# ctu-mrs/space_filling_forest_star

Measured on AMD Instinct MI355X. Metric: accepted node expansions/sec + collision checks/sec, dense_3D 6-DoF, higher is better.
Workload: dtype f64

## Files before the change

### space_filling_forest_star_amd/csrc/devforest.hip

```cpp
#include <hip/hip_runtime.h>
#include <stdint.h>
#include <stdlib.h>
#include "kernels.h"
#include "sff_geom.h"
#include "kernels_dev.h"

namespace sffk {

using namespace sffg;

__device__ __forceinline__ int record_words_dev(int nbcap) { return 6 + 4 * nbcap; }

__device__ __forceinline__ int lemire_pick(unsigned long long word, unsigned long long range) {
  const unsigned long long lo = word * range;
  const unsigned long long hi = __umul64hi(word, range);
  if (lo < range) {
    const unsigned long long thr = (0ULL - range) % range;
    if (lo < thr) return -1;
  }
  return (int)hi;
}

__device__ __forceinline__ int32_t* frontier_now(const DevForestView& f) { return f.ctrl->front_sel ? f.frontier2 : f.frontier; }
__device__ __forceinline__ int32_t* act_now(const DevForestView& f) { return f.ctrl->act_sel ? f.act_slot2 : f.act_slot; }

__device__ void round_begin_scalars(const DevForestView& f, DevCtrl* c) {
  const int cnt = c->act_cnt;
  int n = 0;
  if (c->round < f.threshold_misses && cnt > 0 && c->iter < f.max_iterations && !c->solved) {
    const int left = f.max_iterations - c->iter;
    n = cnt < left ? cnt : left;
  }
  c->n_act = n;
  if (n > 0) {
    if (c->n_nodes + n > f.node_cap - 8 || c->n_borders + n > f.border_cap) {
      c->fault = SFFK_FAULT_CAPACITY;
      c->halt = 1;
      c->n_act = 0;
    } else if ((unsigned long long)(c->n_borders + n) * 2ULL > f.bt_mask + 1ULL) {
      c->fault = SFFK_FAULT_BORDER_TABLE;
      c->halt = 1;
      c->n_act = 0;
    } else {
      c->round += 1;
      c->iter0 = c->iter;
      c->iter += n;
      c->N0 = c->n_nodes;
      c->words_base = c->cursor;
      c->cursor += (unsigned long long)f.words_per * (unsigned long long)n;
      c->rounds += 1;
      c->round_nodes += (unsigned long long)(c->n_nodes + n);
      c->round_queries += (unsigned long long)n;
    }
  }
}

#define WB_BLOCKS 64
__global__ __launch_bounds__(256) void k_wave_begin(DevForestView f) {
  __shared__ int s_last;
  __shared__ int s_scan[4];
  DevCtrl* c = f.ctrl;
  const unsigned long long tb0 = f.profile ? wall_clock64() : 0ULL;
  if (c->halt) {
    if (blockIdx.x == 0 && threadIdx.x == 0) { c->compact_from = 0; c->app_n = 0; }
    return;
  }
  if (c->in_wave) {
    if (blockIdx.x == 0 && threadIdx.x == 0) { c->compact_from = 0; c->app_n = 0; c->ord_valid = 0; round_begin_scalars(f, c); }
    return;
  }
  if (f.prio.n_heaps && !c->empty_frontier) return;
  const bool use_closed = c->closed_n > 0 && c->empty_frontier;
  const int pool = use_closed ? c->closed_n : c->frontier_n;
  int n_slots = f.wave < pool ? f.wave : pool;
  if (n_slots < 1) n_slots = 1;
  const int32_t* from = use_closed ? f.closed : frontier_now(f);
  int32_t* act = act_now(f);
  const unsigned long long cur = c->cursor;
  bool redraw = false;
  for (int sl = blockIdx.x * 256 + threadIdx.x; sl < n_slots; sl += gridDim.x * 256) {
    const unsigned long long wd = f.ring[(cur + (unsigned long long)sl) & f.ring_mask];
    const int pick = lemire_pick(wd, (unsigned long long)pool);
    if (pick < 0) redraw = true;
    else {
      const int node = from[pick];
      f.slot_node[sl] = node; f.slot_pos[sl] = pick;
      if (f.ord.hist) {
        const double* np = f.ord.pos + 6 * (size_t)node;
        const int cx = grid_coord((float)np[0], f.ord.ox, f.ord.inv_cell, f.ord.nx) >> f.ord.shift,
                  cy = grid_coord((float)np[1], f.ord.oy, f.ord.inv_cell, f.ord.ny) >> f.ord.shift,
                  cz = grid_coord((float)np[2], f.ord.oz, f.ord.inv_cell, f.ord.nz) >> f.ord.shift;
        const int key = (cz * f.ord.cny + cy) * f.ord.cnx + cx;
        f.ord.slot_key[sl] = key;
        f.ord.slot_rank[sl] = atomicAdd(&f.ord.hist[key], 1);
      }
    }
    act[sl] = sl;
  }
  if (redraw) atomicOr(&f.commit_seq[2], 1);
  __threadfence();
  __syncthreads();
  if (threadIdx.x == 0) s_last = atomicAdd(&f.commit_seq[1], 1) == (int)gridDim.x - 1;
  __syncthreads();
  if (!s_last) return;
  if (f.ord.hist) {
    constexpr int PERMAX = SFFK_ORD_BUCKETS / 256;
    const int nb = f.ord.n_buckets, per = (nb + 255) >> 8, lane = threadIdx.x & 63, wv = threadIdx.x >> 6;
    int v[PERMAX], sum = 0;
#pragma unroll
    for (int k = 0; k < PERMAX; ++k) {
      const int at = (int)threadIdx.x * per + k;
      v[k] = (k < per && at < nb) ? __hip_atomic_load(&f.ord.hist[at], __ATOMIC_RELAXED, __HIP_MEMORY_SCOPE_AGENT) : 0;
      sum += v[k];
    }
    int inc = sum;
    for (int off = 1; off < 64; off <<= 1) {
      const int o = __shfl_up(inc, off);
      if (lane >= off) inc += o;
    }
    if (lane == 63) s_scan[wv] = inc;
    __syncthreads();
    int run = inc - sum;
    for (int w = 0; w < wv; ++w) run += s_scan[w];
#pragma unroll
    for (int k = 0; k < PERMAX; ++k) {
      const int at = (int)threadIdx.x * per + k;
      if (k < per && at < nb) {
        f.ord.start[at] = run;
        run += v[k];
        f.ord.hist[at] = 0;
      }
    }
  }
  if (threadIdx.x != 0) return;
  c->ord_valid = (f.ord.hist && !__hip_atomic_load(&f.commit_seq[2], __ATOMIC_RELAXED, __HIP_MEMORY_SCOPE_AGENT)) ? 1 : 0;
  unsigned long long used = (unsigned long long)n_slots;
  if (__hip_atomic_load(&f.commit_seq[2], __ATOMIC_RELAXED, __HIP_MEMORY_SCOPE_AGENT)) {
    unsigned long long at = cur;
    for (int s = 0; s < n_slots; ++s) {
      int pick;
      do { pick = lemire_pick(f.ring[at & f.ring_mask], (unsigned long long)pool); ++at; } while (pick < 0);
      f.slot_node[s] = from[pick];
      f.slot_pos[s] = pick;
    }
    used = at - cur;
    c->redraws += 1;
  }
  f.commit_seq[1] = 0;
  f.commit_seq[2] = 0;
  c->compact_from = 0;
  c->app_n = 0;
  c->cursor = cur + used;
  c->n_slots = n_slots;
  c->act_cnt = n_slots;
  c->use_closed = use_closed ? 1 : 0;
  c->round = 0;
  c->in_wave = 1;
  c->waves += 1;
  c->prio_wave = 0;
  c->prio_n0 = c->n_nodes;
  round_begin_scalars(f, c);
  if (f.profile) c->wprof[6] += wall_clock64() - tb0;
}

__device__ __forceinline__ size_t border_slot(const DevForestView& f, unsigned long long key) {
  size_t h = (size_t)((key * 0x9E3779B97F4A7C15ULL) >> 17) & (size_t)f.bt_mask;
  while (true) {
    const unsigned long long cur = f.bt_key[h];
    if (cur == key) return h;
    if (cur == 0ULL) {
      const unsigned long long old = atomicCAS(&f.bt_key[h], 0ULL, key);
      if (old == 0ULL || old == key) return h;
    }
    h = (h + 1) & (size_t)f.bt_mask;
  }
}


#define KC_FAULT_SETTLE() asm volatile("s_waitcnt vmcnt(0)" ::: "memory")
#define KC_SPIN_LIMIT (1 << 20)
#define KC_ACC 0
#define KC_PREF 1
#define KC_WLO 2
#define KC_WHI 3
#define KC_POSTED 4
#define KC_OWN 5
#define KC_CNT 6
#define KC_DEP 12
#define KC_EVN 13

__device__ __forceinline__ unsigned long long kc_load(const unsigned long long* p) {
  return __hip_atomic_load(p, __ATOMIC_RELAXED, __HIP_MEMORY_SCOPE_AGENT);
}
__device__ __forceinline__ void kc_publish(unsigned long long* p, unsigned seq, unsigned v) {
  __hip_atomic_store(p, ((unsigned long long)seq << 32) | (unsigned long long)v, __ATOMIC_RELAXED, __HIP_MEMORY_SCOPE_AGENT);
}
__device__ __forceinline__ unsigned kc_wait(const unsigned long long* p, unsigned seq, int32_t* fault) {
  for (int spin = 0; spin < KC_SPIN_LIMIT; ++spin) {
    const unsigned long long v = kc_load(p);
    if ((unsigned)(v >> 32) == seq) return (unsigned)v;
    __builtin_amdgcn_s_sleep(1);
  }
  atomicOr(fault, 1);
  return 0u;
}
__device__ __forceinline__ unsigned long long kc_block_sum(unsigned long long v, unsigned long long* slot) {
  for (int off = 32; off > 0; off >>= 1) v += __shfl_xor(v, off);
  __syncthreads();
  if (threadIdx.x == 0) *slot = 0ULL;
  __syncthreads();
// ... 430 lines not shown
  }
  __syncthreads();
  for (int w = threadIdx.x; w < (int)(sizeof(DevCtrl) / 4); w += 1024)
    reinterpret_cast<int32_t*>(c)[w] = reinterpret_cast<const int32_t*>(&K)[w];
}

__device__ __forceinline__ void append_ord_store(const ResolveArgs& A, int ord_at, int next) {
  if (ord_at >= 0) (A.f.ctrl->app_act_sel ? A.f.ord.lst[0] : A.f.ord.lst[1])[ord_at] = next;
}
__device__ __forceinline__ int append_one(const ResolveArgs& A, int i, int& slot_out, int& ord_at, int part = 0) {
  ord_at = -1;
  const DevForestView& f = A.f;
  const DevCtrl* c = f.ctrl;
  const int n = c->app_n;
  slot_out = -1;
  if (n <= 0) return -1;
  const int act_cnt = c->app_act_cnt;
  const int32_t* act_old = c->app_act_sel ? f.act_slot2 : f.act_slot;
  int32_t* act_new = c->app_act_sel ? f.act_slot : f.act_slot2;
  const bool wave_over = c->n_act == 0 && !c->halt && c->in_wave && !c->use_closed;
  const bool ord_on = f.ord.hist && c->ord_valid;
  auto claim = [&](int e, int slot) {
    const int nd = f.slot_node[slot];
    atomicMin(&f.claim[nd], e);
    f.ulist[e] = nd;
  };
  if (wave_over && i == 0 && part != 1) f.ctrl->claims_done = 1;
  if (i >= n) {
    if (i < act_cnt && part != 1) {
      const int e = (c->act_cnt - (act_cnt - n)) + (i - n), slot = act_old[i];
      act_new[e] = slot;
      if (wave_over) claim(e, slot);
    }
    return -1;
  }
  const unsigned long long w = f.w_acc[i >> 6];
  const int rank = f.acc_pref[i >> 6] + __popcll(w & ((1ULL << (i & 63)) - 1ULL));
  if (!((w >> (i & 63)) & 1ULL)) {
    auto ord_append = [&](int slot) {
      const int sub = f.ord.slot_pos[slot] >> 6;
      const bool first = c->app_act_sel != 0;
      ord_at = sub * 64 + atomicAdd(&(first ? f.ord.cnt[0] : f.ord.cnt[1])[sub * SFFK_ORD_CNT_STRIDE], 1);
    };
    if (part == 1) {
      if (ord_on) { ord_append(act_old[i]); append_ord_store(A, ord_at, i - rank); }
      return -1;
    }
    slot_out = act_old[i];
    act_new[i - rank] = slot_out;
    if (ord_on && part == 0) ord_append(slot_out);
    if (wave_over) claim(i - rank, slot_out);
    return i - rank;
  }
  if (A.star || part == 2) return -1;
  const int N0 = c->app_N0, fn0 = c->app_fn0;
  int32_t* const frontier = frontier_now(f);
  const int id = N0 + rank;
  const int ex = A.parent[i];
  const double* p = A.newpos + 6 * (size_t)i;
  const size_t o = (size_t)id;
  GridItem it;
  for (int k = 0; k < 6; ++k) it.p[k] = p[k];
  it.id = id;
  it.tree = A.st.tree[ex];
  it.pad[0] = it.pad[1] = 0;
  A.st.x[o] = (float)p[0]; A.st.y[o] = (float)p[1]; A.st.z[o] = (float)p[2];
  A.st.yaw[o] = (float)p[3]; A.st.pitch[o] = (float)p[4]; A.st.roll[o] = (float)p[5];
  for (int k = 0; k < 6; ++k) A.st.pos[6 * o + k] = p[k];
  A.st.tree[o] = it.tree;
  const double pd = A.pdist[i];
  f.parent[o] = ex;
  f.d_closest[o] = pd;
  f.d_root[o] = pd + f.d_root[ex];
  f.iter[o] = (uint32_t)(c->iter0_app + i + 1);
  f.nflag[o] = f.prio.n_heaps ? 0 : 2;
  if (!f.prio.n_heaps) frontier[fn0 + rank] = id;
  grid_put(A.g, it);
  return -1;
}
__device__ void border_finalize(const ResolveArgs& A, int b) {
  __shared__ unsigned long long s_bsum;
  __shared__ int s_bown;
  const DevForestView& f = A.f;
  DevCtrl* c = f.ctrl;
  const int n = c->app_n;
  if (n <= 0 || A.star) return;
  const int nwg = (n + 63) >> 6;
  if (b >= nwg) return;
  const unsigned seq = (unsigned)f.commit_seq[0];
  const unsigned long long stamp_hi = c->epoch << 32;
  const int Tb = f.temp_base, nb0 = c->app_nb0;
  const unsigned long long we = f.w_ev[b];
  unsigned long long* pub = f.wg_pub + (size_t)b * SFFK_PUB_WORDS;
  const int tid = threadIdx.x;
  bool own = false;
  int e_i = 0;
  unsigned long long wo = 0ULL;
  if (tid < 64) {
    if ((we >> tid) & 1ULL) {
      e_i = b * 64 + tid;
      const unsigned long long owner = __hip_atomic_load(&f.bt_val[f.ev_h[e_i]], __ATOMIC_RELAXED, __HIP_MEMORY_SCOPE_AGENT);
      own = owner == (stamp_hi | (unsigned long long)(uint32_t)e_i);
    }
    wo = __ballot(own);
    if (tid == 0) { s_bown = __popcll(wo); kc_publish(pub + KC_OWN, seq, (unsigned)__popcll(wo)); }
  }
  __syncthreads();
  const int n_own = s_bown;
  const bool last = b == nwg - 1;
  if (n_own == 0 && !last) return;
  unsigned long long pe = 0;
  for (int t = tid; t < b; t += 256) pe += kc_wait(f.wg_pub + (size_t)t * SFFK_PUB_WORDS + KC_OWN, seq, f.commit_seq + 6);
  for (int off = 32; off > 0; off >>= 1) pe += __shfl_xor(pe, off);
  if (tid == 0) s_bsum = 0ULL;
  __syncthreads();
  if ((tid & 63) == 0 && pe) atomicAdd(&s_bsum, pe);
  __syncthreads();
  const int ev_pref = (int)s_bsum;
  if (own) {
    const int at = nb0 + ev_pref + __popcll(wo & ((1ULL << tid) - 1ULL));
    double pn[6], pe6[6], dn;
    int ta;
    const int raw = f.ev_raw[e_i], e_nb = f.ev_nb[e_i], e_ex = A.parent[e_i];
    if (raw >= Tb) {
      const int j = raw - Tb;
      for (int q = 0; q < 6; ++q) pn[q] = A.newpos[6 * (size_t)j + q];
      dn = A.pdist[j] + f.d_root[A.parent[j]];
      ta = A.st.tree[A.parent[j]];
    } else {
      for (int q = 0; q < 6; ++q) pn[q] = A.st.pos[6 * (size_t)e_nb + q];
      dn = f.d_root[e_nb];
      ta = A.st.tree[e_nb];
    }
    const int tb = A.st.tree[e_ex];
    f.b_n1[at] = e_nb < e_ex ? e_nb : e_ex; f.b_n2[at] = e_nb < e_ex ? e_ex : e_nb;
    f.b_ta[at] = ta < tb ? ta : tb; f.b_tb[at] = ta < tb ? tb : ta;
    for (int q = 0; q < 6; ++q) pe6[q] = A.st.pos[6 * (size_t)e_ex + q];
    f.b_dist[at] = dn + f.d_root[e_ex] + dist6(pn, pe6);
    f.pair[(size_t)ta * f.n_trees + tb] = 1;
    f.pair[(size_t)tb * f.n_trees + ta] = 1;
  }
  if (last && tid == 0) c->n_borders = nb0 + ev_pref + n_own;
}
__global__ __launch_bounds__(256) void k_append(ResolveArgs A, int append_blocks) {
  if ((int)blockIdx.x >= append_blocks) { border_finalize(A, (int)blockIdx.x - append_blocks); return; }
  int slot, ord_at;
  const int next = append_one(A, blockIdx.x * 256 + threadIdx.x, slot, ord_at);
  append_ord_store(A, ord_at, next);
}
__global__ __launch_bounds__(256) void k_append_sample(ResolveArgs A, SampleLaunch P, int append_blocks) {
  if ((int)blockIdx.x >= 2 * append_blocks) { border_finalize(A, (int)blockIdx.x - 2 * append_blocks); return; }
  const int nb = append_blocks;
  const bool sampler = (int)blockIdx.x >= nb;
  const int tid = ((int)blockIdx.x - (sampler ? nb : 0)) * 256 + threadIdx.x;
  int slot, ord_at;
  if (!sampler) { (void)append_one(A, tid, slot, ord_at, 1); return; }
  const int next = append_one(A, tid, slot, ord_at, 2);
  sample_steer_one(tid, next, slot < 0 ? -2 : slot, P);
  append_ord_store(A, ord_at, next);
}

__device__ void wave_end_control(const DevForestView& f, DevCtrl* c, int removed, int fn, bool from_closed, int n_fail,
                                 const int32_t* grid_ovf, const int32_t* tgrid_ovf, const unsigned long long* star_s) {
  c->closed_n += removed;
  if (f.prio.n_heaps) {
    c->compact_from = 0;
    c->empty_frontier = c->prio_all_empty;
  } else {
    c->compact_from = removed > 0 ? fn : 0;
    c->frontier_n = fn - removed;
    if (removed > 0) c->front_sel ^= 1;
    c->empty_frontier = c->frontier_n == 0 ? 1 : 0;
  }
  if (!c->solved && c->empty_frontier && f.goal_id < 0) {
    const int R = f.n_trees;
    int reached = 1;
    for (int t = 0; t < R; ++t) f.claim[t] = t == 0 ? 1 : 0;
    bool grew = true;
    while (grew) {
      grew = false;
      for (int a = 0; a < R; ++a) {
        if (f.claim[a] != 1) continue;
        f.claim[a] = 2;
        for (int b = 0; b < R; ++b)
          if (f.claim[b] == 0 && f.pair[(size_t)a * R + b]) { f.claim[b] = 1; ++reached; grew = true; }
      }
    }
    for (int t = 0; t < R; ++t) f.claim[t] = 0x7fffffff;
    c->solved = reached == R ? 1 : 0;
  }
  c->claims_done = 0;
  c->clear_n = from_closed ? 0 : n_fail;
  const bool budget = f.node_budget > 0 && c->n_nodes >= f.node_budget;
  c->terminated = (c->solved || c->iter >= f.max_iterations || budget) ? 1 : 0;
  c->halt = c->terminated;
  if (f.commit_seq[6]) { c->fault = SFFK_FAULT_INTERNAL; c->halt = 1; }
  c->in_wave = 0;
  c->n_act = 0;
  c->grid_ovf = grid_ovf[0];
  c->tgrid_ovf = tgrid_ovf[0];
  if (star_s) {
    c->collide_calls += star_s[0]; c->path_free_calls += star_s[1];
    c->star_rounds += star_s[2]; c->star_passes += star_s[3]; c->star_members += star_s[4]; c->star_rewires += star_s[5];
  }
}

#define KW_CNT 15
__device__ void status_publish(const DevForestView& f) {
  if (!f.host_status || threadIdx.x >= 64) return;
  DevCtrl* c = f.ctrl;
  const int sq = __hip_atomic_load(&c->status_seq, __ATOMIC_RELAXED, __HIP_MEMORY_SCOPE_AGENT);
  int32_t* dst = reinterpret_cast<int32_t*>(f.host_status + (sq & (SFFK_STATUS_RING - 1)));
// ... 235 lines not shown
```

### space_filling_forest_star_amd/csrc/devprio.hip

```cpp
#include <hip/hip_runtime.h>
#include <stdint.h>
#include "kernels.h"
#include "sff_geom.h"
#include "kernels_dev.h"
#include "prio_heap_dev.h"

namespace sffk {

using namespace sffg;

__device__ __forceinline__ int prio_lemire(unsigned long long word, unsigned long long range) {
  const unsigned long long lo = word * range;
  const unsigned long long hi = __umul64hi(word, range);
  if (lo < range) {
    const unsigned long long thr = (0ULL - range) % range;
    if (lo < thr) return -1;
  }
  return (int)hi;
}

#ifdef SFFK_PRIO_DEBUG
__device__ unsigned long long g_prio_dbg[16];
#endif
__device__ __forceinline__ int32_t* prio_act_now(const DevForestView& f) { return f.ctrl->act_sel ? f.act_slot2 : f.act_slot; }
// ... 68 lines not shown
  refill();
  auto next_word = [&]() -> unsigned long long {
    if (at - w_lo >= 128ULL) refill();
    const unsigned long long w = s_w[at - w_lo];
    ++at;
    return w;
  };
  auto draw_int = [&](int range) -> int {
    int v;
    do { v = prio_lemire(next_word(), (unsigned long long)range); } while (v < 0);
    return v;
  };
  int32_t* act = prio_act_now(f);
  int made = 0;
  int my_t = 0, my_h = 0, my_i = 0;
  for (int s = 0; s < n_slots; ++s) {
    if (total_ne == 0) break;
    if (at - w_lo >= 96ULL) refill();
    int t;
    do { t = draw_int(T); } while (s_tne[t] == 0);
    const int b0 = P.base[t], nh = P.base[t + 1] - b0;
    int hp;
    do { hp = draw_int(nh); } while (s_sz[b0 + hp] == 0);
    const int size = s_sz[b0 + hp];
    int idx = -1;
    if (!(uniform_real(next_word(), 0.0, 1.0) <= P.bias)) idx = draw_int(size);
    __builtin_amdgcn_wave_barrier();
    if (lane == 0) {
      s_sz[b0 + hp] = size - 1;
      if (size == 1) s_tne[t] -= 1;
    }
    __builtin_amdgcn_wave_barrier();
    if (size == 1) total_ne -= 1;
    if ((s & 63) == lane) { my_t = t; my_h = hp; my_i = idx; }
    if ((s & 63) == 63) {
      const int o = s - 63 + lane;
      P.slot_tree[o] = my_t; P.slot_heap[o] = my_h; P.slot_idx[o] = my_i; act[o] = o;
    }
    ++made;
  }
  if ((made & 63) != 0 && lane < (made & 63)) {
    const int o = (made & ~63) + lane;
    P.slot_tree[o] = my_t; P.slot_heap[o] = my_h; P.slot_idx[o] = my_i; act[o] = o;
  }
  if (lane == 0) {
    c->compact_from = 0;
    c->app_n = 0;
    c->cursor = at;
    c->n_slots = made;
    c->act_cnt = made;
    c->use_closed = 0;
    c->round = 0;
    c->in_wave = 1;
    c->waves += 1;
    c->prio_wave = 1;
    c->prio_gen = (int32_t)c->waves;
    c->prio_n0 = c->n_nodes;
    prio_round_begin(f, c);
  }
}


#define PP_COIN_WORDS ((4 * 64 * SFFK_DEV_MAX_GROUPS + 4096) / 32)
__global__ __launch_bounds__(1024) void k_prio_plan(DevForestView f) {
  __shared__ int s_sz[SFFK_PRIO_MAX_HEAPS];
  __shared__ int s_cnt[SFFK_PRIO_MAX_HEAPS];
  __shared__ unsigned int s_coin[PP_COIN_WORDS];
  __shared__ int s_fn[1024][4];
  __shared__ int s_bad, s_pool, s_used;
  DevCtrl* c = f.ctrl;
  const PrioView& P = f.prio;
  const int tid = threadIdx.x, lane = tid & 63;
  if (c->halt || c->in_wave || !P.plan) return;
  const int H = P.n_heaps, T = f.n_trees;
  for (int h = tid; h < H; h += 1024) { s_sz[h] = P.size[h]; s_cnt[h] = 0; }
  if (tid == 0) { s_bad = 0; s_pool = 0; s_used = -1; }
  __syncthreads();
  if (tid < T && P.base[tid + 1] > P.base[tid]) atomicAdd(&s_pool, s_sz[P.base[tid]]);
  __syncthreads();
  int n_slots = f.wave < s_pool ? f.wave : s_pool;
  if (n_slots < 1) n_slots = 1;
  const int M = 4 * n_slots + 8;
  int bk = (M + 1023) / 1024;
  if (bk < 4) bk = 4;
  const int span = 1024 * bk + 64;
  const unsigned long long cur = c->cursor;
  for (int p0 = 0; p0 < span; p0 += 8 * 1024) {
    unsigned long long w[8];
    for (int j = 0; j < 8; ++j) {
      const int p = p0 + j * 1024 + tid;
      w[j] = f.ring[(cur + (unsigned long long)(p < M ? p : M - 1)) & f.ring_mask];
    }
    for (int j = 0; j < 8; ++j) {
      const int p = p0 + j * 1024 + tid;
      const bool coin = p < M && !(uniform_real(w[j], 0.0, 1.0) <= P.bias);
      const unsigned long long m = __ballot(coin);
      if (lane == 0 && p < span && (p >> 5) + 1 < PP_COIN_WORDS) { s_coin[p >> 5] = (unsigned int)m; s_coin[(p >> 5) + 1] = (unsigned int)(m >> 32); }
    }
  }
  __syncthreads();
  auto hop = [&](int p) -> int { return p + 3 + (int)((s_coin[(p + 2) >> 5] >> ((p + 2) & 31)) & 1u); };
  const int lo = tid * bk, hi = lo + bk;
  for (int e = 0; e < 4; ++e) {
    int p = lo + e, n = 0;
    while (p < hi) { p = hop(p); ++n; }
    s_fn[tid][e] = (n << 2) | (p - hi);
// ... 2 lines not shown
  for (int d = 1; d < 1024; d <<= 1) {
    int g[4];
    for (int e = 0; e < 4; ++e) g[e] = s_fn[tid][e];
    if (tid >= d) {
      int r[4];
      for (int e = 0; e < 4; ++e) {
        const int first = s_fn[tid - d][e];
        const int then = g[first & 3];
        r[e] = (((first >> 2) + (then >> 2)) << 2) | (then & 3);
      }
      for (int e = 0; e < 4; ++e) g[e] = r[e];
    }
    __syncthreads();
    for (int e = 0; e < 4; ++e) s_fn[tid][e] = g[e];
    __syncthreads();
  }
  int p = lo, s = 0;
  if (tid > 0) { const int before = s_fn[tid - 1][0]; p = lo + (before & 3); s = before >> 2; }
  int32_t* act = prio_act_now(f);
  while (p < hi && s <= n_slots) {
    if (s == n_slots) { s_used = p; break; }
    const unsigned long long w0 = f.ring[(cur + (unsigned long long)p) & f.ring_mask];
    const unsigned long long w1 = f.ring[(cur + (unsigned long long)p + 1ULL) & f.ring_mask];
    const int nx = hop(p);
    bool bad = false;
    int t = prio_lemire(w0, (unsigned long long)T), hp = 0, idx = -1;
    unsigned long long w3 = 0ULL;
    if (t < 0) { bad = true; t = 0; }
    else {
      const int b0 = P.base[t], nh = P.base[t + 1] - b0;
      hp = nh > 0 ? prio_lemire(w1, (unsigned long long)nh) : -1;
      if (hp < 0) { bad = true; hp = 0; }
      else {
        atomicAdd(&s_cnt[b0 + hp], 1);
        if (nx - p == 4) { idx = -2; w3 = f.ring[(cur + (unsigned long long)p + 3ULL) & f.ring_mask]; }
      }
    }
    if (bad) s_bad = 1;
    P.slot_tree[s] = t; P.slot_heap[s] = hp; P.slot_idx[s] = idx; P.slot_word[s] = w3; act[s] = s;
    p = nx; ++s;
  }
  __syncthreads();
  for (int h = tid; h < H; h += 1024) if (s_cnt[h] > s_sz[h]) s_bad = 1;
  __syncthreads();
  if (s_bad || s_used < 0 || tid != 0) return;
  c->compact_from = 0;
  c->app_n = 0;
  c->cursor = cur + (unsigned long long)s_used;
  c->n_slots = n_slots;
  c->act_cnt = n_slots;
  c->use_closed = 0;
  c->round = 0;
  c->in_wave = 1;
  c->waves += 1;
  c->prio_wave = 1;
  c->prio_gen = (int32_t)c->waves;
  c->prio_n0 = c->n_nodes;
  prio_round_begin(f, c);
}

#define PG_CHUNK 2048
__device__ __forceinline__ int block_excl_scan_256(int v, int* s_w, int* total) {
  const int lane = threadIdx.x & 63, w = threadIdx.x >> 6;
  int x = v;
  for (int d = 1; d < 64; d <<= 1) { const int y = __shfl_up(x, d); if (lane >= d) x += y; }
  __syncthreads();
  if (lane == 63) s_w[w] = x;
  __syncthreads();
  int before = 0, sum = 0;
  for (int i = 0; i < 4; ++i) { if (i < w) before += s_w[i]; sum += s_w[i]; }
  *total = sum;
  return before + x - v;
}

__global__ __launch_bounds__(256) void k_prio_pops(DevForestView f) {
  __shared__ int s_slot[PG_CHUNK];
  __shared__ int s_idx[PG_CHUNK];
  __shared__ unsigned long long s_word[PG_CHUNK];
  __shared__ int s_w[4];
  const DevCtrl* c = f.ctrl;
  const PrioView& P = f.prio;
  const int h = blockIdx.x, tid = threadIdx.x, lane = tid & 63;
  if (!c->prio_wave || !c->in_wave || P.gen[h] == c->prio_gen) return;
  int t = 0;
  while (P.base[t + 1] <= h) ++t;
  const int hp = h - P.base[t];
  const int n_slots = c->n_slots;
  HeapRef hr = heap_of(P, h);
  for (int c0 = 0; c0 < n_slots; c0 += PG_CHUNK) {
    int st_[8], sh_[8];
    for (int j = 0; j < 8; ++j) {
      const int s = c0 + tid * 8 + j;
      const int sc = s < n_slots ? s : n_slots - 1;
      const int a_ = P.slot_tree[sc], b_ = P.slot_heap[sc];
      st_[j] = s < n_slots ? a_ : -1;
      sh_[j] = s < n_slots ? b_ : -1;
    }
    int cnt = 0;
    for (int j = 0; j < 8; ++j) cnt += (st_[j] == t && sh_[j] == hp) ? 1 : 0;
    int total;
    int at = block_excl_scan_256(cnt, s_w, &total);
    for (int j = 0; j < 8; ++j)
      if (st_[j] == t && sh_[j] == hp) {
        const int s = c0 + tid * 8 + j;
        const int idx = P.slot_idx[s];
        s_slot[at] = s; s_idx[at] = idx; s_word[at] = idx == -2 ? P.slot_word[s] : 0ULL;
// ... 160 lines not shown
```

### space_filling_forest_star_amd/csrc/kernels.h

```cpp
#pragma once
#include <hip/hip_runtime.h>
#include <stdint.h>

#include "knobs.h"

namespace sffk {

struct NodeStoreView {
  const float* x;
  const float* y;
  const float* z;
  const float* yaw;
  const float* pitch;
  const float* roll;
  const int32_t* tree;
  const double* pos;
};

struct NodeStoreMut {
  float *x, *y, *z, *yaw, *pitch, *roll;
  int32_t* tree;
  double* pos;
};

// ... 73 lines not shown
  int clear_n[3];
  const int32_t* tg_start;
  const int32_t* tg_list;
  double tg_org[3];
  double tg_inv;
  int tg_n[3];
};
void launch_tgrid_build(hipStream_t s, const EnvView& env, int32_t* cnt_or_start, int32_t* list, bool fill);
struct ClearBuildArgs {
  double thr_pose, thr_edge;
  double pose_lo[3], pose_hi[3];
  double edge_lo[3], edge_hi[3];
};
void launch_clear_build(hipStream_t s, const EnvView& env, const ClearBuildArgs& P, uint32_t* bits_pose, uint32_t* bits_edge,
                        long long n_cells);

struct RobotView {
  const double* tri;
  int n_tri;
  double center[3];
  double radius;
  double lo[3], hi[3];
};

struct DevCtrl {
  int32_t n_act;
  int32_t halt;
  int32_t n_nodes, iter, round, in_wave;
  int32_t n_slots, frontier_n, closed_n, use_closed;
  int32_t terminated, solved, empty_frontier, fault;
  int32_t N0, iter0, n_borders, n_unsettled;
  int32_t fault_pending, redraws, grid_ovf, tgrid_ovf;
  int32_t front_sel;
  int32_t compact_from;
  int32_t act_sel, act_cnt;
  int32_t app_n, app_N0, app_fn0, app_act_sel;
  int32_t iter0_app, app_act_cnt;
  int32_t claims_done;
  int32_t clear_n;
  unsigned long long cursor;
  unsigned long long words_base;
  unsigned long long collide_calls, path_free_calls, nn_queries;
  unsigned long long poses_executed, segments_executed, samples_executed;
  unsigned long long waves, rounds, round_nodes, round_queries;
  unsigned long long epoch;
  unsigned long long work_items;
  unsigned long long prof[8];
  unsigned long long q_t0, q_t1, q_ticks, q_launches;
  unsigned long long wprof[8];
  int32_t prio_n0, prio_wave, prio_all_empty, prio_gen;
  unsigned long long star_rounds, star_passes, star_members, star_rewires;
  int32_t ord_valid;
  int32_t app_nb0;
  int32_t status_seq, status_pad;
  unsigned long long spec_steps, spec_evaluated, spec_committed;
  int32_t spec_stalled, spec_pad;
};
#define SFFK_STATUS_RING 4
#define SFFK_DEV_MAX_GROUPS 1024
#define SFFK_FAULT_LISTS 1
#define SFFK_FAULT_BORDER_TABLE 2
#define SFFK_FAULT_CAPACITY 4
#define SFFK_FAULT_INTERNAL 16
#define SFFK_FAULT_PRIO_REDRAW 8

#define SFFK_ORD_BUCKETS 4096
#define SFFK_ORD_CNT_STRIDE 32
struct OrderView {
  int32_t* hist;
  int32_t* start;
  int32_t* slot_key;
  int32_t* slot_rank;
  int32_t* slot_pos;
  int32_t* lst[2];
  int32_t* cnt[2];
  int32_t n_sub;
  const double* pos;
  float ox, oy, oz, inv_cell;
  int32_t nx, ny, nz, shift, cnx, cny;
  int32_t n_buckets;
};

struct DevRound {
  const DevCtrl* ctrl;
  const int32_t* act_slot;
  const int32_t* act_slot2;
  const int32_t* slot_node;
  const uint8_t* nflag;
  const uint64_t* ring;
  uint64_t ring_mask;
  const double* trig;
  int32_t words_per;
  int32_t* parent_out;
  uint8_t* force_out;
  unsigned long long* qclk;
  unsigned long long* qclk_sh;
  OrderView ord;
};

struct RoundTemps {
  GridView tg;
  NodeStoreMut st;
  int32_t* cnt;
  int32_t* ctrl;
  int32_t* sub;
  int n_perm;
  int base;
// ... 370 lines not shown
```

### space_filling_forest_star_amd/csrc/kernels.hip

```cpp
#include <hip/hip_runtime.h>
#include <stdint.h>
#include <stdlib.h>
#include <string.h>
#include "kernels.h"
#include <algorithm>
#include "sff_geom.h"
#include "kernels_dev.h"
#include "star_pass_dev.h"
#include "prio_heap_dev.h"

namespace sffk {

using namespace sffg;


__global__ __launch_bounds__(256) void k_sample_steer(SampleLaunch P) {
  const int i = blockIdx.x * blockDim.x + threadIdx.x;
  sample_steer_one(i, i, -1, P);
}

__device__ __forceinline__ float wrapf(float d) {
  const float PI_F = 3.14159274f;
  if (d < -PI_F) return d + 2.0f * PI_F;
  if (d >= PI_F) return d - 2.0f * PI_F;
  return d;
}

__global__ __launch_bounds__(256) void k_sweep(NodeStoreView st, int first, int n_nodes,
                                               const SweepQuery* __restrict__ queries,
                                               const double* __restrict__ qpos,
                                               int nq, int q_per_block, int32_t* __restrict__ cnt,
                                               int32_t* __restrict__ hit_idx, double* __restrict__ hit_dist, int cap) {
  const int n4 = (n_nodes + 3) >> 2;
  const int q_begin = blockIdx.y * q_per_block;
  const int q_end = q_begin + q_per_block < nq ? q_begin + q_per_block : nq;
  for (int t = blockIdx.x * blockDim.x + threadIdx.x; t < n4; t += gridDim.x * blockDim.x) {
    const int base = first + (t << 2);
    const int t4 = (first >> 2) + t;
    float4 X = reinterpret_cast<const float4*>(st.x)[t4];
    float4 Y = reinterpret_cast<const float4*>(st.y)[t4];
    float4 Z = reinterpret_cast<const float4*>(st.z)[t4];
    float4 A = reinterpret_cast<const float4*>(st.yaw)[t4];
    float4 B = reinterpret_cast<const float4*>(st.pitch)[t4];
    float4 C = reinterpret_cast<const float4*>(st.roll)[t4];
    const float xs[4] = {X.x, X.y, X.z, X.w}, ys[4] = {Y.x, Y.y, Y.z, Y.w}, zs[4] = {Z.x, Z.y, Z.z, Z.w};
    const float as[4] = {A.x, A.y, A.z, A.w}, bs[4] = {B.x, B.y, B.z, B.w}, cs[4] = {C.x, C.y, C.z, C.w};
    for (int q = q_begin; q < q_end; ++q) {
      const SweepQuery Q = queries[q];
      if (!Q.active) continue;
      float d3[4];
      bool any = false;
#pragma unroll
      for (int j = 0; j < 4; ++j) {
        float dx = xs[j] - Q.x, dy = ys[j] - Q.y, dz = zs[j] - Q.z;
        d3[j] = fmaf(dz, dz, fmaf(dy, dy, dx * dx));
        any |= d3[j] <= Q.r2f;
      }
      if (!any) continue;
#pragma unroll
      for (int j = 0; j < 4; ++j) {
        const int id = base + j;
        if (!(d3[j] <= Q.r2f) || id >= first + n_nodes || id >= Q.max_id) continue;
        float da = wrapf(as[j] - Q.yaw), db = wrapf(bs[j] - Q.pitch), dc = wrapf(cs[j] - Q.roll);
        float d6 = fmaf(dc, dc, fmaf(db, db, fmaf(da, da, d3[j])));
        if (!(d6 <= Q.r2f)) continue;
        if (Q.tree >= 0 ? st.tree[id] != Q.tree : (Q.tree < -1 && st.tree[id] == -2 - Q.tree)) continue;
        double np[6], qp[6];
        for (int k = 0; k < 6; ++k) { np[k] = st.pos[6 * (size_t)id + k]; qp[k] = qpos[6 * (size_t)q + k]; }
        double d = dist6(np, qp);
        if (d < Q.r) {
          int slot = atomicAdd(&cnt[q], 1);
// ... 5443 lines not shown
```

### space_filling_forest_star_amd/csrc/kernels_dev.h

```cpp
#pragma once
#include <hip/hip_runtime.h>
#include <stdint.h>
#include "kernels.h"
#include "sff_geom.h"

namespace sffk {

__device__ __forceinline__ int grid_coord(float v, float o, float inv, int n) {
  float f = floorf((v - o) * inv);
  int c = f < 0.0f ? 0 : (f > (float)(n - 1) ? n - 1 : (int)f);
  return c;
}

__device__ __forceinline__ size_t grid_cell_of(const GridView& g, float x, float y, float z) {
  const int cx = grid_coord(x, g.ox, g.inv_cell, g.nx), cy = grid_coord(y, g.oy, g.inv_cell, g.ny),
            cz = grid_coord(z, g.oz, g.inv_cell, g.nz);
  return ((size_t)cz * g.ny + cy) * g.nx + cx;
}
__device__ __forceinline__ void grid_put(const GridView& g, const GridItem& it) {
  const size_t cell = grid_cell_of(g, (float)it.p[0], (float)it.p[1], (float)it.p[2]);
  const int slot = atomicAdd(g.cnt + cell, 1);
  if (g.occ) atomicOr(g.occ + (cell >> 5), 1u << (cell & 31));
  GridItem32 lt;
  lt.x = (float)it.p[0]; lt.y = (float)it.p[1]; lt.z = (float)it.p[2];
// ... 91 lines not shown
  if (lane < have) {
    const unsigned long long bits = a_on ? (((unsigned long long)(unsigned)a_hi << 32) | (unsigned)a_lo) : (((unsigned long long)(unsigned)b_hi << 32) | (unsigned)b_lo);
    t.d = __longlong_as_double((long long)bits);
    t.id = a_on ? a_id : b_id;
  } else { t.d = 1.0e300; t.id = 0x7fffffff; }
}
__device__ __forceinline__ double topk_worst(const TopK& t, int k, int have) {
  return have < k ? 1.0e300 : __shfl(t.d, k - 1);
}

__device__ __forceinline__ bool star_accepted(const DevForestView& f, int i, int& rank) {
  const unsigned long long w = f.w_acc[i >> 6];
  rank = f.acc_pref[i >> 6] + __popcll(w & ((1ULL << (i & 63)) - 1ULL));
  return (w >> (i & 63)) & 1ULL;
}

__device__ __forceinline__ void star_cells_mates(const GridView& tg, int m, int cell, int lane, const double* qp, int tree, int Tb,
                                                 int self, double limit, const DevForestView& f, TopK& t, int k, int& have) {
  int inc = m;
  for (int off = 1; off < 64; off <<= 1) {
    const int o = __shfl_up(inc, off);
    if (lane >= off) inc += o;
  }
  const int total = __shfl(inc, 63);
  for (int base = 0; base < total; base += 64) {
    const int j = base + lane;
    const int jj = j < total ? j : total - 1;
    int lo = 0, hi = 63;
    while (lo < hi) {
      const int mid = (lo + hi) >> 1;
      if (__shfl(inc, mid) > jj) hi = mid; else lo = mid + 1;
    }
    const int src_cell = __shfl(cell, lo);
    const int slot = jj - (__shfl(inc, lo) - __shfl(m, lo));
    bool cand = false;
    double d = 1.0e300;
    int id = 0x7fffffff;
    if (j < total) {
      const GridItem it = tg.items[(size_t)src_cell * tg.bk + slot];
      id = it.id;
      int rk;
      if (it.tree == tree && id >= Tb && id < self && star_accepted(f, id - Tb, rk)) {
        d = sffg::dist6(it.p, qp);
        cand = d <= limit;
      }
    }
    const double worst = topk_worst(t, k, have);
    cand = cand && (have < k || key_less(d, id, worst, 0x7fffffff));
    topk_insert(t, lane, k, have, __ballot(cand), d, id);
  }
}


__device__ __forceinline__ void sample_steer_one(int tid, int i, int slot, const SampleLaunch& P) {
  using namespace sffg;
  const uint64_t* __restrict__ words = P.words;
  const int32_t* __restrict__ parent = P.parent;
  const double* __restrict__ node_pos = P.node_pos;
  const double* __restrict__ center_in = P.center_in;
  int n = P.n;
  const double dist = P.dist;
  const int dim = P.dim;
  const SampleParams& prm = P.prm;
  double* __restrict__ out6 = P.out6;
  uint8_t* __restrict__ in_lim = P.in_lim;
  double* __restrict__ parent_dist = P.parent_dist;
  SweepQuery* __restrict__ queries = P.queries;
  const int32_t q_max_base = P.q_max_base;
  const RoundTemps& tmp = P.tmp;
  const DevRound& dv = P.dv;
  if (dv.ctrl) {
    if (dv.ctrl->halt) return;
    n = dv.ctrl->n_act;
    if (tid == 0 && dv.qclk) { dv.qclk[0] = ~0ULL; dv.qclk[1] = 0ULL; }
    if (dv.qclk_sh && tid < 128) dv.qclk_sh[(tid >> 1) * 16 + (tid & 1)] = (tid & 1) ? ~0ULL : 0ULL;
  }
  if (tmp.cnt) {
    if (tid < n) tmp.cnt[tid] = 0;
    if (tid < 32) tmp.ctrl[tid] = 0;
    if (tmp.sub && tid < SFFK_SUBLISTS) {
      tmp.sub[tid * SFFK_SUB_STRIDE] = 0; tmp.sub[tid * SFFK_SUB_STRIDE + 1] = 0; tmp.sub[tid * SFFK_SUB_STRIDE + 2] = 0;
    }
    if (tid < tmp.base - tmp.n_perm) {
      const float nanv = __int_as_float(0x7fc00000);
      const size_t o = (size_t)tmp.n_perm + tid;
      tmp.st.x[o] = nanv; tmp.st.y[o] = nanv; tmp.st.z[o] = nanv;
      tmp.st.yaw[o] = nanv; tmp.st.pitch[o] = nanv; tmp.st.roll[o] = nanv;
    }
  }
  if (dv.ctrl && dv.ord.hist && slot == -1 && dv.ctrl->ord_valid && dv.ctrl->round == 1 && tid < dv.ctrl->n_slots) {
    const int pos = dv.ord.start[dv.ord.slot_key[tid]] + dv.ord.slot_rank[tid];
    const int sel = dv.ctrl->act_sel, n_slots = dv.ctrl->n_slots;
    dv.ord.slot_pos[tid] = pos;
    (sel ? dv.ord.lst[1] : dv.ord.lst[0])[pos] = tid < n ? tid : -1;
    if ((pos & 63) == 0) (sel ? dv.ord.cnt[1] : dv.ord.cnt[0])[(pos >> 6) * SFFK_ORD_CNT_STRIDE] = n_slots - pos < 64 ? n_slots - pos : 64;
  }
  if (i < 0 || i >= n) return;
  double c[6], o[6];
  int par = 0;
  if (dv.ctrl) {
    par = dv.slot_node[slot >= 0 ? slot : (dv.ctrl->act_sel ? dv.act_slot2 : dv.act_slot)[i]];
    dv.parent_out[i] = par;
    dv.force_out[i] = dv.nflag[par] & 1;
  } else if (!center_in) {
    par = parent[i];
  }
  const double* src = center_in ? center_in + 6 * (size_t)i : node_pos + 6 * (size_t)par;
  for (int k = 0; k < 6; ++k) c[k] = src[k];
  if (tmp.center_out) for (int k = 0; k < 6; ++k) tmp.center_out[6 * (size_t)i + k] = c[k];
  uint64_t w[6];
  SampleTrig host_trig{};
  if (dv.ctrl) {
    const unsigned long long base = dv.ctrl->words_base + (unsigned long long)dv.words_per * (unsigned long long)i;
    for (int k = 0; k < 6; ++k) w[k] = k < dv.words_per ? dv.ring[(base + k) & dv.ring_mask] : 0ULL;
    if (dv.trig) {
      const double* t0 = dv.trig + 3 * (size_t)(base & dv.ring_mask);
      host_trig.c_phi = t0[0]; host_trig.s_phi = t0[1];
      if (dv.words_per == 6) {
        const double* t1 = dv.trig + 3 * (size_t)((base + 1) & dv.ring_mask);
        const double* t3 = dv.trig + 3 * (size_t)((base + 3) & dv.ring_mask);
        host_trig.c_theta = t1[0]; host_trig.s_theta = t1[1];
        host_trig.acos_u = t3[2];
      }
    }
  } else {
    for (int k = 0; k < 6; ++k) w[k] = words[6 * (size_t)i + k];
  }
  bool ok;
  if (dv.ctrl && dv.trig) {
    ok = sample_point_with(w, c, dist, dim, prm.limits, o, host_trig);
  } else if (tmp.preset) {
    for (int k = 0; k < 6; ++k) o[k] = tmp.preset[6 * (size_t)i + k];
    ok = in_limits(o, prm.limits);
  } else {
    ok = sample_point(w, c, dist, dim, prm.limits, o);
  }
  for (int k = 0; k < 6; ++k) out6[6 * (size_t)i + k] = o[k];
  in_lim[i] = ok ? 1 : 0;
  if (tmp.cnt) {
    const float nanv = __int_as_float(0x7fc00000);
    const size_t t = (size_t)tmp.base + i;
    tmp.st.x[t] = ok ? (float)o[0] : nanv;
    tmp.st.y[t] = ok ? (float)o[1] : nanv;
    tmp.st.z[t] = ok ? (float)o[2] : nanv;
    tmp.st.yaw[t] = ok ? (float)o[3] : nanv;
    tmp.st.pitch[t] = ok ? (float)o[4] : nanv;
    tmp.st.roll[t] = ok ? (float)o[5] : nanv;
    for (int k = 0; k < 6; ++k) tmp.st.pos[6 * t + k] = o[k];
    const int tr = tmp.st.tree[par];
    tmp.st.tree[t] = tr;
    if (ok && tmp.tg.cnt) {
      GridItem it;
      for (int k = 0; k < 6; ++k) it.p[k] = o[k];
      it.id = (int32_t)t;
      it.tree = tr;
      it.pad[0] = it.pad[1] = 0;
      grid_put(tmp.tg, it);
    }
  }
  if (parent_dist) {
    double pd = dist6(c, o);
    parent_dist[i] = pd;
    if (queries) {
      SweepQuery q;
      q.x = (float)o[0]; q.y = (float)o[1]; q.z = (float)o[2];
      q.yaw = (float)o[3]; q.pitch = (float)o[4]; q.roll = (float)o[5];
      double r = pd > prm.dist_tree ? pd : prm.dist_tree;
      q.r = r;
      double ri = (r + prm.sweep_abs_eps) * (1.0 + 1e-5);
      q.r2f = (float)(ri * ri) * 1.000001f;
      q.tree = -1;
      q.max_id = q_max_base + i;
      q.active = (ok && (prm.world <= 1 || i % prm.world == prm.rank)) ? 1 : 0;
      q.pad = 0;
      queries[i] = q;
      if (tmp.qrec) {
        QRec r;
        r.q[0] = q.x; r.q[1] = q.y; r.q[2] = q.z; r.q[3] = q.yaw; r.q[4] = q.pitch; r.q[5] = q.roll;
        r.r2f = q.r2f; r.max_id = q.max_id; r.q_tree = q.tree;
        r.mine = tmp.cnt ? tmp.st.tree[par] : 0;
        r.evaluate = q.active;
        const GridView& g = tmp.tg;
        const float rf = sqrtf(q.r2f) * 1.000001f;
        const int lx = grid_coord(q.x - rf, g.ox, g.inv_cell, g.nx), hx = grid_coord(q.x + rf, g.ox, g.inv_cell, g.nx);
        const int ly = grid_coord(q.y - rf, g.oy, g.inv_cell, g.ny), hy = grid_coord(q.y + rf, g.oy, g.inv_cell, g.ny);
        const int lz = grid_coord(q.z - rf, g.oz, g.inv_cell, g.nz), hz = grid_coord(q.z + rf, g.oz, g.inv_cell, g.nz);
        r.lx = lx; r.ly = ly; r.lz = lz; r.wx = hx - lx + 1; r.wy = hy - ly + 1;
        r.total = q.active ? r.wx * r.wy * (hz - lz + 1) : 0;
        const double parts0 = pd / 0.1;
        r.ns0 = edge_samples(parts0);
        const float inv0 = (float)tmp.clear_inv * __frcp_rn((float)parts0);
        for (int k = 0; k < 3; ++k) {
          r.t0[k] = (float)((c[k] - tmp.clear_org[k]) * tmp.clear_inv);
          r.t0[3 + k] = (float)(o[k] - c[k]) * inv0;
        }
        r.pdist = pd; r.qr = q.r;
        r.scratch[0] = r.scratch[1] = r.scratch[2] = r.scratch[3] = 0;
        tmp.qrec[i] = r;
      }
    }
  }
}

}
```

Measured before the change: 11.14 million.

## Split sampler into fetch/finish phases and speculatively issue control and index loads

The sampling path is restructured into a control snapshot, a fetch phase and a finish phase. Control scalars, active-slot indices and parent ids are loaded speculatively up front and pinned with empty inline-asm barriers, so the dependent global loads are issued together instead of serialised behind the halt/n_act reads. A new act_identity flag lets the first round skip the act_slot indirection, and the fused append+sample path gets a dedicated list builder that computes compaction indices and claims directly. This adds code complexity and relies on the clamped speculative loads being in bounds and on the identity invariant holding.

```diff
diff --git a/profiles/small_wave_legs.py b/profiles/small_wave_legs.py
--- /dev/null
+++ b/profiles/small_wave_legs.py
@@ -0,0 +1,30 @@
+import json
+import os
+import sys
+import time
+
+ROOT = os.path.dirname(os.path.dirname(os.path.abspath(__file__)))
+sys.path.insert(0, ROOT)
+sys.path.insert(0, os.path.join(ROOT, "tests"))
+
+import common
+import space_filling_forest_star_amd as S
+
+sc = common.scenario("dense3d")
+ctx = S.Context(0)
+ctx.upload_env(sc["env"])
+ctx.upload_robot(sc["robot"])
+roots = common.free_roots(lambda p: int(ctx.collide_poses(p[None, :])[0]), sc["limits"], 10, seed=1)
+out = {"lib": os.environ.get("SFFGPU_LIB", "libsffgpu.so")}
+for wave, iters in ((64, 150000), (512, 1000000)):
+    for n in (iters // 10, iters):
+        f = S.Forest(ctx, roots, sc["limits"], dist_tree=sc["dist_tree"], sampling_dist=sc["sampling_dist"], dim=6,
+                     max_iterations=n, node_budget=0, wave=wave, seed=1)
+        t0 = time.perf_counter()
+        f.run()
+        dt = time.perf_counter() - t0
+        st, dev = f.stats(), bool(f.device_engine())
+        f.close()
+    out["wave_%d" % wave] = {"iterations_per_s": st["iterations"] / dt, "iterations": st["iterations"], "nodes": st["n_nodes"],
+                             "device_engine": dev, "seconds": dt}
+print(json.dumps(out), flush=True)
diff --git a/space_filling_forest_star_amd/csrc/devforest.hip b/space_filling_forest_star_amd/csrc/devforest.hip
--- a/space_filling_forest_star_amd/csrc/devforest.hip
+++ b/space_filling_forest_star_amd/csrc/devforest.hip
@@ -66,7 +66,7 @@
     return;
   }
   if (c->in_wave) {
-    if (blockIdx.x == 0 && threadIdx.x == 0) { c->compact_from = 0; c->app_n = 0; c->ord_valid = 0; round_begin_scalars(f, c); }
+    if (blockIdx.x == 0 && threadIdx.x == 0) { c->compact_from = 0; c->app_n = 0; c->ord_valid = 0; c->act_identity = 0; round_begin_scalars(f, c); }
     return;
   }
   if (f.prio.n_heaps && !c->empty_frontier) return;
@@ -156,6 +156,7 @@
   c->use_closed = use_closed ? 1 : 0;
   c->round = 0;
   c->in_wave = 1;
+  c->act_identity = 1;
   c->waves += 1;
   c->prio_wave = 0;
   c->prio_n0 = c->n_nodes;
@@ -692,7 +693,7 @@
     if (wave_over) claim(i - rank, slot_out);
     return i - rank;
   }
-  if (A.star || part == 2) return -1;
+  if (A.star) return -1;
   const int N0 = c->app_N0, fn0 = c->app_fn0;
   int32_t* const frontier = frontier_now(f);
   const int id = N0 + rank;
@@ -788,16 +789,57 @@
   const int next = append_one(A, blockIdx.x * 256 + threadIdx.x, slot, ord_at);
   append_ord_store(A, ord_at, next);
 }
+__device__ __forceinline__ int append_list_one(const ResolveArgs& A, int i, int bound, int& par, SampleCtl& K) {
+  const DevForestView& f = A.f;
+  const DevCtrl* c = f.ctrl;
+  const int ic = i < bound ? i : bound - 1;
+  unsigned long long w = f.w_acc[ic >> 6];
+  int pref = f.acc_pref[ic >> 6];
+  int s0 = f.act_slot[ic], s1 = f.act_slot2[ic];
+  int ex = A.parent[ic];
+  K = sample_ctl(c);
+  int n = c->app_n, act_cnt = c->app_act_cnt, app_sel = c->app_act_sel, new_cnt = c->act_cnt;
+  int in_wave = c->in_wave, use_closed = c->use_closed;
+  join_ctl_v(K);
+  join_v(n, act_cnt, app_sel, new_cnt, in_wave, use_closed, w, pref, s0, s1, ex);
+  const bool wave_over = K.n == 0 && !K.halt && in_wave && !use_closed;
+  par = 0;
+  if (n <= 0) return -1;
+  const int slot = app_sel ? s1 : s0;
+  int32_t* act_new = app_sel ? f.act_slot : f.act_slot2;
+  if (wave_over && i == 0) f.ctrl->claims_done = 1;
+  if (i >= n) {
+    if (i < act_cnt) {
+      const int e = (new_cnt - (act_cnt - n)) + (i - n);
+      act_new[e] = slot;
+      if (wave_over) { const int nd = f.slot_node[slot]; atomicMin(&f.claim[nd], e); f.ulist[e] = nd; }
+    }
+    return -1;
+  }
+  if ((w >> (i & 63)) & 1ULL) return -1;
+  const int next = i - (pref + __popcll(w & ((1ULL << (i & 63)) - 1ULL)));
+  par = ex;
+  act_new[next] = slot;
+  if (wave_over) { atomicMin(&f.claim[ex], next); f.ulist[next] = ex; }
+  return next;
+}
 __global__ __launch_bounds__(256) void k_append_sample(ResolveArgs A, SampleLaunch P, int append_blocks) {
   if ((int)blockIdx.x >= 2 * append_blocks) { border_finalize(A, (int)blockIdx.x - 2 * append_blocks); return; }
   const int nb = append_blocks;
   const bool sampler = (int)blockIdx.x >= nb;
   const int tid = ((int)blockIdx.x - (sampler ? nb : 0)) * 256 + threadIdx.x;
-  int slot, ord_at;
-  if (!sampler) { (void)append_one(A, tid, slot, ord_at, 1); return; }
-  const int next = append_one(A, tid, slot, ord_at, 2);
-  sample_steer_one(tid, next, slot < 0 ? -2 : slot, P);
-  append_ord_store(A, ord_at, next);
+  if (!sampler) {
+    int slot, ord_at;
+    (void)append_one(A, tid, slot, ord_at, 1);
+    return;
+  }
+  int par;
+  SampleCtl K;
+  const int next = append_list_one(A, tid, P.n, par, K);
+  if (K.halt) return;
+  const bool valid = next >= 0 && next < K.n;
+  const SampleIn S = sample_fetch(valid ? next : 0, valid ? par : 0, K, P);
+  sample_finish(tid, valid, next, par, S, -1, K, P);
 }
 
 __device__ void wave_end_control(const DevForestView& f, DevCtrl* c, int removed, int fn, bool from_closed, int n_fail,
diff --git a/space_filling_forest_star_amd/csrc/devprio.hip b/space_filling_forest_star_amd/csrc/devprio.hip
--- a/space_filling_forest_star_amd/csrc/devprio.hip
+++ b/space_filling_forest_star_amd/csrc/devprio.hip
@@ -144,6 +144,7 @@
     c->use_closed = 0;
     c->round = 0;
     c->in_wave = 1;
+    c->act_identity = 1;
     c->waves += 1;
     c->prio_wave = 1;
     c->prio_gen = (int32_t)c->waves;
@@ -252,6 +253,7 @@
   c->use_closed = 0;
   c->round = 0;
   c->in_wave = 1;
+  c->act_identity = 1;
   c->waves += 1;
   c->prio_wave = 1;
   c->prio_gen = (int32_t)c->waves;
diff --git a/space_filling_forest_star_amd/csrc/kernels.h b/space_filling_forest_star_amd/csrc/kernels.h
--- a/space_filling_forest_star_amd/csrc/kernels.h
+++ b/space_filling_forest_star_amd/csrc/kernels.h
@@ -149,7 +149,8 @@
   unsigned long long star_rounds, star_passes, star_members, star_rewires;
   int32_t ord_valid;
   int32_t app_nb0;
-  int32_t status_seq, status_pad;
+  int32_t status_seq;
+  int32_t act_identity;
   unsigned long long spec_steps, spec_evaluated, spec_committed;
   int32_t spec_stalled, spec_pad;
 };
diff --git a/space_filling_forest_star_amd/csrc/kernels.hip b/space_filling_forest_star_amd/csrc/kernels.hip
--- a/space_filling_forest_star_amd/csrc/kernels.hip
+++ b/space_filling_forest_star_amd/csrc/kernels.hip
@@ -16,7 +16,7 @@
 
 __global__ __launch_bounds__(256) void k_sample_steer(SampleLaunch P) {
   const int i = blockIdx.x * blockDim.x + threadIdx.x;
-  sample_steer_one(i, i, -1, P);
+  sample_steer_one(i, P);
 }
 
 __device__ __forceinline__ float wrapf(float d) {
diff --git a/space_filling_forest_star_amd/csrc/kernels_dev.h b/space_filling_forest_star_amd/csrc/kernels_dev.h
--- a/space_filling_forest_star_amd/csrc/kernels_dev.h
+++ b/space_filling_forest_star_amd/csrc/kernels_dev.h
@@ -167,13 +167,62 @@
 }
 
 
-__device__ __forceinline__ void sample_steer_one(int tid, int i, int slot, const SampleLaunch& P) {
+struct SampleCtl {
+  int32_t n, halt, act_sel, round, ord_valid, n_slots, act_identity;
+  unsigned long long words_base;
+};
+__device__ __forceinline__ SampleCtl sample_ctl(const DevCtrl* c) {
+  SampleCtl K;
+  K.n = c->n_act; K.halt = c->halt; K.act_sel = c->act_sel; K.round = c->round; K.ord_valid = c->ord_valid;
+  K.n_slots = c->n_slots; K.act_identity = c->act_identity; K.words_base = c->words_base;
+  return K;
+}
+template <class T> __device__ __forceinline__ void join_one_u(T& x) { asm volatile("" : "+s"(x) : : "memory"); }
+template <class T> __device__ __forceinline__ void join_one_v(T& x) { asm volatile("" : "+v"(x) : : "memory"); }
+template <class... T> __device__ __forceinline__ void join_u(T&... x) { (join_one_u(x), ...); }
+template <class... T> __device__ __forceinline__ void join_v(T&... x) { (join_one_v(x), ...); }
+__device__ __forceinline__ void join_ctl_u(SampleCtl& K) {
+  join_u(K.n, K.halt, K.act_sel, K.round, K.ord_valid, K.n_slots, K.act_identity, K.words_base);
+}
+__device__ __forceinline__ void join_ctl_v(SampleCtl& K) {
+  join_v(K.n, K.halt, K.act_sel, K.round, K.ord_valid, K.n_slots, K.act_identity, K.words_base);
+}
+struct SampleIn {
+  double c[6];
+  uint64_t w[6];
+  sffg::SampleTrig trig;
+  int32_t tree;
+  uint8_t force;
+};
+__device__ __forceinline__ SampleIn sample_fetch(int i, int par, const SampleCtl& K, const SampleLaunch& P) {
+  const DevRound& dv = P.dv;
+  SampleIn S{};
+  const double* src = P.center_in ? P.center_in + 6 * (size_t)i : P.node_pos + 6 * (size_t)par;
+  for (int k = 0; k < 6; ++k) S.c[k] = src[k];
+  if (P.tmp.cnt) S.tree = P.tmp.st.tree[par];
+  if (dv.ctrl) {
+    S.force = dv.nflag[par] & 1;
+    const unsigned long long base = K.words_base + (unsigned long long)dv.words_per * (unsigned long long)i;
+    for (int k = 0; k < 6; ++k) S.w[k] = k < dv.words_per ? dv.ring[(base + k) & dv.ring_mask] : 0ULL;
+    if (dv.trig) {
+      const double* t0 = dv.trig + 3 * (size_t)(base & dv.ring_mask);
+      S.trig.c_phi = t0[0]; S.trig.s_phi = t0[1];
+      if (dv.words_per == 6) {
+        const double* t1 = dv.trig + 3 * (size_t)((base + 1) & dv.ring_mask);
+        const double* t3 = dv.trig + 3 * (size_t)((base + 3) & dv.ring_mask);
+        S.trig.c_theta = t1[0]; S.trig.s_theta = t1[1];
+        S.trig.acos_u = t3[2];
+      }
+    }
+  } else {
+    for (int k = 0; k < 6; ++k) S.w[k] = P.words[6 * (size_t)i + k];
+  }
+  return S;
+}
+__device__ __forceinline__ void sample_finish(int tid, bool valid, int i, int par, const SampleIn& S, int ord_pos,
+                                              const SampleCtl& K, const SampleLaunch& P) {
   using namespace sffg;
-  const uint64_t* __restrict__ words = P.words;
-  const int32_t* __restrict__ parent = P.parent;
-  const double* __restrict__ node_pos = P.node_pos;
-  const double* __restrict__ center_in = P.center_in;
-  int n = P.n;
+  const int n = K.n;
   const double dist = P.dist;
   const int dim = P.dim;
   const SampleParams& prm = P.prm;
@@ -185,8 +234,6 @@
   const RoundTemps& tmp = P.tmp;
   const DevRound& dv = P.dv;
   if (dv.ctrl) {
-    if (dv.ctrl->halt) return;
-    n = dv.ctrl->n_act;
     if (tid == 0 && dv.qclk) { dv.qclk[0] = ~0ULL; dv.qclk[1] = 0ULL; }
     if (dv.qclk_sh && tid < 128) dv.qclk_sh[(tid >> 1) * 16 + (tid & 1)] = (tid & 1) ? ~0ULL : 0ULL;
   }
@@ -203,47 +250,24 @@
       tmp.st.yaw[o] = nanv; tmp.st.pitch[o] = nanv; tmp.st.roll[o] = nanv;
     }
   }
-  if (dv.ctrl && dv.ord.hist && slot == -1 && dv.ctrl->ord_valid && dv.ctrl->round == 1 && tid < dv.ctrl->n_slots) {
-    const int pos = dv.ord.start[dv.ord.slot_key[tid]] + dv.ord.slot_rank[tid];
-    const int sel = dv.ctrl->act_sel, n_slots = dv.ctrl->n_slots;
+  if (ord_pos >= 0) {
+    const int sel = K.act_sel, n_slots = K.n_slots, pos = ord_pos;
     dv.ord.slot_pos[tid] = pos;
     (sel ? dv.ord.lst[1] : dv.ord.lst[0])[pos] = tid < n ? tid : -1;
     if ((pos & 63) == 0) (sel ? dv.ord.cnt[1] : dv.ord.cnt[0])[(pos >> 6) * SFFK_ORD_CNT_STRIDE] = n_slots - pos < 64 ? n_slots - pos : 64;
   }
-  if (i < 0 || i >= n) return;
+  if (!valid) return;
   double c[6], o[6];
-  int par = 0;
+  uint64_t w[6];
+  for (int k = 0; k < 6; ++k) { c[k] = S.c[k]; w[k] = S.w[k]; }
   if (dv.ctrl) {
-    par = dv.slot_node[slot >= 0 ? slot : (dv.ctrl->act_sel ? dv.act_slot2 : dv.act_slot)[i]];
     dv.parent_out[i] = par;
-    dv.force_out[i] = dv.nflag[par] & 1;
-  } else if (!center_in) {
-    par = parent[i];
-  }
-  const double* src = center_in ? center_in + 6 * (size_t)i : node_pos + 6 * (size_t)par;
-  for (int k = 0; k < 6; ++k) c[k] = src[k];
+    dv.force_out[i] = S.force;
+  }
   if (tmp.center_out) for (int k = 0; k < 6; ++k) tmp.center_out[6 * (size_t)i + k] = c[k];
-  uint64_t w[6];
-  SampleTrig host_trig{};
-  if (dv.ctrl) {
-    const unsigned long long base = dv.ctrl->words_base + (unsigned long long)dv.words_per * (unsigned long long)i;
-    for (int k = 0; k < 6; ++k) w[k] = k < dv.words_per ? dv.ring[(base + k) & dv.ring_mask] : 0ULL;
-    if (dv.trig) {
-      const double* t0 = dv.trig + 3 * (size_t)(base & dv.ring_mask);
-      host_trig.c_phi = t0[0]; host_trig.s_phi = t0[1];
-      if (dv.words_per == 6) {
-        const double* t1 = dv.trig + 3 * (size_t)((base + 1) & dv.ring_mask);
-        const double* t3 = dv.trig + 3 * (size_t)((base + 3) & dv.ring_mask);
-        host_trig.c_theta = t1[0]; host_trig.s_theta = t1[1];
-        host_trig.acos_u = t3[2];
-      }
-    }
-  } else {
-    for (int k = 0; k < 6; ++k) w[k] = words[6 * (size_t)i + k];
-  }
   bool ok;
   if (dv.ctrl && dv.trig) {
-    ok = sample_point_with(w, c, dist, dim, prm.limits, o, host_trig);
+    ok = sample_point_with(w, c, dist, dim, prm.limits, o, S.trig);
   } else if (tmp.preset) {
     for (int k = 0; k < 6; ++k) o[k] = tmp.preset[6 * (size_t)i + k];
     ok = in_limits(o, prm.limits);
@@ -252,6 +276,7 @@
   }
   for (int k = 0; k < 6; ++k) out6[6 * (size_t)i + k] = o[k];
   in_lim[i] = ok ? 1 : 0;
+  const int tr = S.tree;
   if (tmp.cnt) {
     const float nanv = __int_as_float(0x7fc00000);
     const size_t t = (size_t)tmp.base + i;
@@ -262,7 +287,6 @@
     tmp.st.pitch[t] = ok ? (float)o[4] : nanv;
     tmp.st.roll[t] = ok ? (float)o[5] : nanv;
     for (int k = 0; k < 6; ++k) tmp.st.pos[6 * t + k] = o[k];
-    const int tr = tmp.st.tree[par];
     tmp.st.tree[t] = tr;
     if (ok && tmp.tg.cnt) {
       GridItem it;
@@ -293,7 +317,7 @@
         QRec r;
         r.q[0] = q.x; r.q[1] = q.y; r.q[2] = q.z; r.q[3] = q.yaw; r.q[4] = q.pitch; r.q[5] = q.roll;
         r.r2f = q.r2f; r.max_id = q.max_id; r.q_tree = q.tree;
-        r.mine = tmp.cnt ? tmp.st.tree[par] : 0;
+        r.mine = tr;
         r.evaluate = q.active;
         const GridView& g = tmp.tg;
         const float rf = sqrtf(q.r2f) * 1.000001f;
@@ -317,4 +341,32 @@
   }
 }
 
-}
+__device__ __forceinline__ void sample_steer_one(int tid, const SampleLaunch& P) {
+  const DevRound& dv = P.dv;
+  const int tc = tid < P.n ? tid : P.n - 1;
+  SampleCtl K{};
+  K.n = P.n;
+  int par = 0, a0 = 0, a1 = 0, key = 0, rnk = 0;
+  if (dv.ctrl) {
+    const int32_t* kp = dv.ord.hist ? dv.ord.slot_key : dv.act_slot;
+    const int32_t* rp = dv.ord.hist ? dv.ord.slot_rank : dv.act_slot;
+    a0 = dv.act_slot[tc]; a1 = dv.act_slot2[tc];
+    par = dv.slot_node[tc];
+    key = kp[tc]; rnk = rp[tc];
+    K = sample_ctl(dv.ctrl);
+    join_ctl_u(K);
+    join_v(a0, a1, par, key, rnk);
+  } else if (!P.center_in) {
+    par = P.parent[tc];
+  }
+  if (K.halt) return;
+  const bool valid = tid < K.n;
+  if (dv.ctrl && !(K.act_identity && K.round == 1)) par = dv.slot_node[valid ? (K.act_sel ? a1 : a0) : 0];
+  if (!valid) par = 0;
+  const bool ord_now = dv.ctrl && dv.ord.hist && K.ord_valid && K.round == 1 && tid < K.n_slots;
+  const SampleIn S = sample_fetch(valid ? tid : 0, par, K, P);
+  const int start = dv.ctrl && dv.ord.hist ? dv.ord.start[ord_now ? key : 0] : 0;
+  sample_finish(tid, valid, tid, par, S, ord_now ? start + rnk : -1, K, P);
+}
+
+}
```

Result: faster. 11.27 million, median of 6 (+1.1%).
